# fanzhongyi/ExploreMultiModal

Hardware: AMD Instinct MI355X
Metric: image-text pairs/sec fwd+bwd, VLMo-Base, 1/2/4/8 MI355X; % bf16 MFMA roofline (higher is better)
Workload: dtype bf16

## Files before the change

exploremultimodal_amd/csrc/block.hip:

```cpp
#include "common.h"
#include "vlmo_hip.h"
#include <algorithm>
#include <map>
#include <vector>

namespace {
constexpr int GELU_DERIV = 4;


struct Events {
    std::vector<hipEvent_t> pool;
    hipEvent_t get(size_t i) {
        while (pool.size() <= i) {
            hipEvent_t e = nullptr;
            (void)hipEventCreateWithFlags(&e, hipEventDisableTiming);
            pool.push_back(e);
        }
        return pool[i];
    }
};
Events& events() {
    static thread_local std::map<int, Events> per_device;
    int dev = 0;
    (void)hipGetDevice(&dev);
// ... 152 lines not shown
    VLMO_CHECK_ARG(b->dx2 && b->dx1 && b->dx0, "vlmo_stack_bwd: block %d: null gradient buffers", i);
    VLMO_CHECK_ARG(b->n_experts >= 1 && b->n_experts <= 2 && b->n_attn >= 1 && b->n_attn <= 2,
                   "vlmo_stack_bwd: block %d: 1..2 experts and attention launches per block", i);
    VLMO_CHECK_ARG(b->M > 0 && b->exp_rows[0] >= 0 && (b->n_experts == 1 || b->exp_rows[1] >= 0) &&
                       (int64_t)b->exp_rows[0] + (b->n_experts == 2 ? b->exp_rows[1] : 0) <= b->M,
                   "vlmo_stack_bwd: block %d: expert rows exceed M = %d", i, b->M);
    const int64_t need = stack_ws_layout(b->M, b->d, b->hidden, block_seqs(b)).total * 4;
    VLMO_CHECK_ARG(b->ws_main && b->ws_bytes >= need,
                   "vlmo_stack_bwd: block %d: column workspace of %lld bytes is too small: need %lld bytes = "
                   "vlmo_stack_bwd_ws_bytes(%d, %d, %d, %d)",
                   i, (long long)b->ws_bytes, (long long)need, b->M, b->d, b->hidden, block_seqs(b));
    return 0;
}

int block_dgrad_chain(const VlmoBlockDesc* b, hipStream_t st, Deferred& D, const VlmoBlockDesc* below, bool skip_resid,
                      bool* fused_below) {
    const int M = b->M, d = b->d, hid = b->hidden;
    const int nseq_all = block_seqs(b);
    const StackWs W = stack_ws_layout(M, d, hid, nseq_all);
    const int64_t slot_bytes = W.slot * 4;
    float* const ws = b->ws_main;
    const void *ag[4], *wg[4], *af[4], *wf[4];
    int32_t rows[4];
    VlmoEpilogue eg[4], ef[4];
    float* colpart = ws + W.colpart;
    for (int x = 0; x < b->n_experts; ++x) {
        const size_t r0 = b->exp_row0[x];
        const int n = rows[x] = b->exp_rows[x];
        if (!skip_resid) {
            VlmoColJob fold{};
            TRY(resid_bwd_launch(b->dx2 + r0 * d, bp(b->zd2, r0, d, 2), b->g2,
// ... 49 lines not shown
                          b->dqkv, qvsum + (size_t)s0 * 2 * d, b->heads, d, b->maxlen[a], scale, b->attn_drop_thresh,
                          b->attn_inv_keep, b->seed + 11 + b->attn_seed_idx[a], b->attn_seq0[a], st));
    push_tn(D, b->dz1, d, b->ctx, d, b->dproj_w, d, M, d, d);
    push_tn(D, b->dqkv, 3 * d, b->y1, d, b->dqkv_w, d, M, 3 * d, d);
    push_col(D, fold_job(qvsum, 2 * d, nseq_all, 2 * d, d, b->dqkv_b, b->dqkv_b + 2 * d));
    {
        VlmoEpilogue e = epi();
        e.out = b->dy1;
        e.ldo = d;
        TRY(vlmo_gemm_nt(VLMO_EPI_BIAS, VLMO_BF16, b->tile, b->dqkv, 3 * d, b->qkv_wT, 3 * d, M, d, 3 * d, &e, st));
    }
    const VlmoBlockDesc* n = below;
    *fused_below = n && n->M == M && n->d == d && n->dx2 == b->dx0 && n->zd2 && n->dz2 && n->exp_row0[0] == 0 &&
                   (n->n_experts == 1 ? n->exp_rows[0] == M
                                      : (n->exp_row0[1] == n->exp_rows[0] && n->exp_rows[0] + n->exp_rows[1] == M));
    VlmoColJob fold{};
    if (*fused_below) {
        const int seg = n->n_experts == 1 ? M : n->exp_row0[1];
        float* wsf = ws + W.ln1;
        int nb0 = 0;
        TRY(ln_resid_seg_bwd(b->dy1, b->x, b->n1w, b->mean1, b->rstd1, b->dx1, b->dx0, b->dn1w, b->dn1b, n->zd2, n->g2,
                             n->rs2, n->row_index, n->dz2, n->dg2, n->drop_thresh, n->inv_keep, n->seed + 21, n->seed + 23,
                             seg, M, d, wsf, 2 * slot_bytes, &fold, &nb0, st));
        push_col(D, fold);
        if (n->db2[0]) push_col(D, fold_job(wsf + 3 * d, 4 * d, nb0, d, d, n->db2[0]));
        if (n->n_experts == 2 && n->db2[1])
            push_col(D, fold_job(wsf + 3 * d + (size_t)nb0 * 4 * d, 4 * d, fold.rows - nb0, d, d, n->db2[1]));
    } else {
        TRY(ln_bwd_fold(b->dy1, b->x, b->n1w, b->mean1, b->rstd1, b->dx1, b->dx0, b->dn1w, b->dn1b, nullptr, nullptr, nullptr,
                        nullptr, nullptr, nullptr, nullptr, 0, 1.f, 0, M, d, ws + W.ln1, slot_bytes, &fold, st));
        push_col(D, fold);
    }
    return 0;
}

}

extern "C" int64_t vlmo_stack_bwd_ws_bytes(int M, int d, int hidden, int max_seqs) {
    return stack_ws_layout(M, d, hidden, max_seqs).total * 4;
}

extern "C" int vlmo_stack_fwd(const VlmoStackDesc* s, hipStream_t st) {
    VLMO_CHECK_ARG(s && s->blocks && s->n_blocks >= 1, "vlmo_stack_fwd: empty stack");
    for (int i = 0; i < s->n_blocks; ++i)
        if (int rc = block_fwd(&s->blocks[i], st)) return rc;
    return 0;
}

extern "C" int vlmo_stack_bwd(const VlmoStackDesc* s, hipStream_t st) {
    VLMO_CHECK_ARG(s && s->blocks && s->n_blocks >= 1, "vlmo_stack_bwd: empty stack");
    const int nb = s->n_blocks;
    for (int i = 0; i < nb; ++i) TRY(check_block_bwd(&s->blocks[i], i));
    const int batch = s->wgrad_batch >= 1 ? s->wgrad_batch : 1;
    const int nsets = s->n_tmp_sets >= 1 ? s->n_tmp_sets : 1;
    hipStream_t side = s->side_stream ? s->side_stream : st;
    const bool two = side != st;
    VLMO_CHECK_ARG(!two || nsets > batch || nb <= nsets,
                   "vlmo_stack_bwd: %d temporary sets cannot cover deferred batches of %d blocks", nsets, batch);
    Events& ev = events();
    Deferred D;
    D.store = s->wgrad_store != 0;
    std::vector<int> batch_of(nb, -1);
    int n_batches = 0, waited_upto = -1;
    auto flush = [&]() -> int {
        if (D.blocks.empty()) return 0;
        if (two) {
            hipEvent_t f = ev.get(2 * n_batches);
            (void)hipEventRecord(f, st);
            (void)hipStreamWaitEvent(side, f, 0);
        }
        std::stable_sort(D.tn.begin(), D.tn.end(), [](const VlmoTnProblem& a, const VlmoTnProblem& b) { return a.M > b.M; });
        TRY(vlmo_gemm_tn_multi(VLMO_BF16, D.tn.data(), (int)D.tn.size(), side));
        TRY(vlmo_colwork_multi(VLMO_BF16, D.col.data(), (int)D.col.size(), side));
        if (two) (void)hipEventRecord(ev.get(2 * n_batches + 1), side);
        if (s->grad_ready)
            for (int i : D.blocks)
                if (s->grad_ready[i]) (void)hipEventRecord((hipEvent_t)s->grad_ready[i], side);
        ++n_batches;
        D.tn.clear();
        D.col.clear();
        D.blocks.clear();
        return 0;
    };
    auto set_free = [&](int kk) -> int {
        if (!two || kk < nsets || kk >= nb) return 0;
        int need = batch_of[kk - nsets];
        if (need < 0 || need >= n_batches) {
            TRY(flush());
            need = n_batches - 1;
        }
        if (need >= 0 && need > waited_upto) {
            (void)hipStreamWaitEvent(st, ev.get(2 * need + 1), 0);
            waited_upto = need;
        }
        return 0;
    };
    bool skip_resid = false;
    for (int k = 0; k < nb; ++k) {
        const int i = nb - 1 - k;
        TRY(set_free(k));
        TRY(set_free(k + 1));
        bool fused = false;
        TRY(block_dgrad_chain(&s->blocks[i], st, D, i > 0 ? &s->blocks[i - 1] : nullptr, skip_resid, &fused));
        skip_resid = fused;
        D.blocks.push_back(i);
        batch_of[k] = n_batches;
        if ((int)D.blocks.size() >= batch || k == nb - 1) TRY(flush());
    }
    if (two && n_batches > 0) (void)hipStreamWaitEvent(st, ev.get(2 * (n_batches - 1) + 1), 0);
    return 0;
}

extern "C" int vlmo_event_create(void** out) {
    VLMO_CHECK_ARG(out, "vlmo_event_create: null out");
    hipEvent_t e = nullptr;
    hipError_t rc = hipEventCreateWithFlags(&e, hipEventDisableTiming);
    if (rc != hipSuccess) {
        vlmo_set_error("vlmo_event_create: %s", hipGetErrorString(rc));
        return (int)rc;
    }
    *out = e;
    return 0;
// ... 7 lines not shown
```

exploremultimodal_amd/csrc/gemm_tn.hip:

```cpp
#include "gemm_common.h"
#include <algorithm>
#include <vector>

namespace {

struct GemmTN {
    const void* A;
    const void* B;
    float* C;
    int M, N1, N2, lda, ldb, ldc;
    int kt_per_split, tiles;
    float alpha;
    float* slab;
    int mode;
};
enum { TN_ATOMIC = 0, TN_ACCUM = 1, TN_STORE = 2 };

__device__ __attribute__((aligned(256))) char tn_zero_page[256];

__device__ __forceinline__ int tn_swz(int row) { return ((row & 3) << 2) | ((row >> 2) & 3); }

template <typename T, int BM, int BN, int WM, int WN, bool PP = false>
__device__ __forceinline__ void gemm_tn_body(const GemmTN& p, const int lid) {
    typedef typename Elem<T>::v8 v8;
// ... 225 lines not shown
                        p.slab[((size_t)split * p.N1 + gm) * p.N2 + gn] = acc[i][j][r];
                    else if (p.mode == TN_STORE)
                        *c = p.alpha * acc[i][j][r];
                    else
                        atomicAdd(c, p.alpha * acc[i][j][r]);
                }
            }
        }
}

template <typename T, int BM, int BN, int WM, int WN, bool PP = false>
__global__ __launch_bounds__(WM * WN * 64, 2) void gemm_tn_kernel(const GemmTN p) {
    gemm_tn_body<T, BM, BN, WM, WN, PP>(p, xcd_remap(blockIdx.x, gridDim.x));
}

constexpr int MAX_TN_PROBS = 16;
constexpr int MAX_TN_ORDER = 1024;
constexpr uint16_t TN_NOP = 0xFFFF;
struct GemmTNMulti {
    int n;
    GemmTN p[MAX_TN_PROBS];
    uint16_t order[MAX_TN_ORDER];
};
template <typename T>
__global__ __launch_bounds__(512, 2) void gemm_tn_multi_kernel(const GemmTNMulti mp) {
    const uint32_t code = mp.order[blockIdx.x];
    if (code == TN_NOP) return;
    int gi = (int)(code >> 12);
    const int lid_in = __builtin_amdgcn_readfirstlane((int)(code & 0xFFFu));
    gi = __builtin_amdgcn_readfirstlane(gi);
    const GemmTN& q = mp.p[gi];
    GemmTN p;
    p.A = uniform_ptr(q.A), p.B = uniform_ptr(q.B), p.C = (float*)uniform_ptr(q.C);
    p.M = __builtin_amdgcn_readfirstlane(q.M), p.N1 = __builtin_amdgcn_readfirstlane(q.N1);
    p.N2 = __builtin_amdgcn_readfirstlane(q.N2), p.lda = __builtin_amdgcn_readfirstlane(q.lda);
    p.ldb = __builtin_amdgcn_readfirstlane(q.ldb), p.ldc = __builtin_amdgcn_readfirstlane(q.ldc);
    p.kt_per_split = __builtin_amdgcn_readfirstlane(q.kt_per_split), p.tiles = __builtin_amdgcn_readfirstlane(q.tiles);
    p.alpha = __builtin_bit_cast(float, __builtin_amdgcn_readfirstlane(__builtin_bit_cast(int, q.alpha)));
    p.slab = nullptr;
    p.mode = __builtin_amdgcn_readfirstlane(q.mode);
    gemm_tn_body<T, 256, 256, 2, 4, true>(p, lid_in);
}

__global__ __launch_bounds__(256) void tn_reduce_kernel(const float* __restrict__ slab, int splits, int N1, int N2,
                                                        float* __restrict__ C, int ldc, float alpha) {
    const int n4 = N2 >> 2;
// ... 21 lines not shown
    int splits = splits_req;
    if (splits <= 0) {
        if (pl.big) {
            splits = 256 / pl.tiles;
        } else {
            splits = 512 / pl.tiles;
            if (splits < 4) splits = 1024 / pl.tiles;
        }
        if (splits < 1) splits = 1;
    }
    if (splits > nk) splits = nk;
    pl.per = (nk + splits - 1) / splits;
    pl.splits = (nk + pl.per - 1) / pl.per;
    return pl;
}
}

extern "C" int64_t vlmo_gemm_tn_ws_bytes(int M, int N1, int N2) {
    const TnPlan a = tn_plan(M, N1, N2, 0, 0);
    return (int64_t)a.splits * N1 * N2 * 4;
}

extern "C" int vlmo_gemm_tn(int dtype, const void* A, int lda, const void* B, int ldb, float* C, int ldc,
                            int M, int N1, int N2, float alpha, int splits, float* ws, int64_t ws_bytes,
                            hipStream_t stream) {
    VLMO_CHECK_ARG(A && B && C, "vlmo_gemm_tn: null operand");
    VLMO_CHECK_ARG(M > 0 && N1 >= 8 && N2 >= 8, "vlmo_gemm_tn: bad problem M=%d N1=%d N2=%d", M, N1, N2);
    VLMO_CHECK_ARG(N1 % 8 == 0 && N2 % 8 == 0 && lda % 8 == 0 && ldb % 8 == 0, "vlmo_gemm_tn: N1,N2,lda,ldb must be multiples of 8");
    VLMO_CHECK_ARG(lda >= N1 && ldb >= N2 && ldc >= N2, "vlmo_gemm_tn: leading dimension too small");
    VLMO_CHECK_ARG(dtype == VLMO_BF16 || dtype == VLMO_F16, "vlmo_gemm_tn: dtype must be bf16 or f16");
// ... 54 lines not shown
        }
        long tiles_all = 0;
        int min_nk = 1 << 30;
        double flops = 0;
        for (int q = 0; q < nq; ++q) {
            const VlmoTnProblem& r = probs[q0 + q];
            VLMO_CHECK_ARG(r.A && r.B && r.C, "vlmo_gemm_tn_multi: null operand in problem %d", q0 + q);
            VLMO_CHECK_ARG(r.M > 0 && r.N1 >= 8 && r.N2 >= 8 && r.N1 % 8 == 0 && r.N2 % 8 == 0 && r.lda % 8 == 0 &&
                               r.ldb % 8 == 0 && r.lda >= r.N1 && r.ldb >= r.N2 && r.ldc >= r.N2,
                           "vlmo_gemm_tn_multi: bad shape in problem %d (M=%d N1=%d N2=%d)", q0 + q, r.M, r.N1, r.N2);
            tiles_all += (long)((r.N1 + 255) / 256) * ((r.N2 + 255) / 256);
            const int nk = (r.M + 63) / 64;
            if (nk < min_nk) min_nk = nk;
            flops += 2.0 * r.M * r.N1 * r.N2;
        }
        int splits = 1;
        if (tiles_all < 192) {
            splits = (int)(256 / tiles_all);
            if (splits > min_nk / 8) splits = min_nk / 8;
            if (splits < 1) splits = 1;
        }
        GemmTNMulti mp{};
        mp.n = nq;
        struct Job {
            uint16_t code;
            int cost;
        };
        std::vector<Job> jobs;
        for (int q = 0; q < nq; ++q) {
            const VlmoTnProblem& r = probs[q0 + q];
            const int tiles = ((r.N1 + 255) / 256) * ((r.N2 + 255) / 256);
            const int nk = (r.M + 63) / 64;
            int sp = splits > nk ? nk : splits;
            const int per = (nk + sp - 1) / sp;
            sp = (nk + per - 1) / per;
            int mode = r.accumulate ? TN_ACCUM : TN_STORE;
            if (sp > 1) {
                mode = TN_ATOMIC;
                if (!r.accumulate) {
                    hipError_t rc = hipMemset2DAsync(r.C, (size_t)r.ldc * 4, 0, (size_t)r.N2 * 4, r.N1, stream);
                    if (rc != hipSuccess) {
                        vlmo_set_error("vlmo_gemm_tn_multi: memset failed: %s", hipGetErrorString(rc));
                        return (int)rc;
                    }
                }
            }
            VLMO_CHECK_ARG(tiles * sp <= 4096, "vlmo_gemm_tn_multi: problem %d has too many tiles", q0 + q);
            mp.p[q] = GemmTN{r.A, r.B, r.C, r.M, r.N1, r.N2, r.lda, r.ldb, r.ldc, per, tiles, r.alpha, nullptr, mode};
            for (int l = 0; l < tiles * sp; ++l) jobs.push_back(Job{(uint16_t)((q << 12) | l), per});
        }
        std::stable_sort(jobs.begin(), jobs.end(), [](const Job& a, const Job& b) { return a.cost > b.cost; });
        std::vector<uint16_t> bins[8];
        for (size_t i = 0; i < jobs.size();) {
            size_t j = i;
            while (j < jobs.size() && jobs[j].cost == jobs[i].cost) ++j;
            const size_t cnt = j - i;
            for (int x = 0; x < 8; ++x)
                for (size_t k = i + cnt * x / 8; k < i + cnt * (x + 1) / 8; ++k) bins[x].push_back(jobs[k].code);
            i = j;
        }
        size_t deepest = 0;
        for (int x = 0; x < 8; ++x) deepest = bins[x].size() > deepest ? bins[x].size() : deepest;
        VLMO_CHECK_ARG(deepest * 8 <= (size_t)MAX_TN_ORDER, "vlmo_gemm_tn_multi: %zu workgroups exceed one launch (pass fewer problems per call)",
                       jobs.size());
        const int t = (int)deepest * 8;
        for (int b = 0; b < t; ++b) {
            const std::vector<uint16_t>& bin = bins[b & 7];
            mp.order[b] = (size_t)(b >> 3) < bin.size() ? bin[b >> 3] : TN_NOP;
        }
        ProfScope prof(73, flops, stream);
        constexpr int LDS = 2 * 4 * 64 * 256;
        if (dtype == VLMO_F16)
            hipLaunchKernelGGL((gemm_tn_multi_kernel<f16>), dim3(t), dim3(512), LDS, stream, mp);
        else
// ... 6 lines not shown
```

exploremultimodal_amd/engine.py:

```python
import ctypes
import os as _os
import sys
from collections import namedtuple

import torch

from . import hip

LN_EPS = 1e-12
GRAD_SINK = None
_ov = _os.environ.get('VLMO_OVERLAP_WGRAD')
OVERLAP_WGRAD = None if _ov is None else _ov != '0'
ONE_STREAM_ROWS = 12288


def _use_side_stream(sink, rows):
    if OVERLAP_WGRAD is not None:
        return OVERLAP_WGRAD
    return sink is not None or rows < ONE_STREAM_ROWS


DEFAULT_TILE = -1


# ... 421 lines not shown

def wgrad_batch_for(d, hid, cus=256, max_batch=4):
    if WGRAD_BATCH > 0:
        return WGRAD_BATCH
    c = lambda n: -(-n // 256)
    tiles = c(d) * c(3 * d) + c(d) * c(d) + 2 * c(d) * c(hid)
    best, best_cost = 1, None
    for b in range(1, max_batch + 1):
        cost = -(-b * tiles // cus) / b
        if best_cost is None or cost < best_cost - 1e-9:
            best, best_cost = b, cost
    return best


TMP_SETS = 4
USE_STACK = True

_PERSIST = {}


def _persist(dev, tag, numel, dtype):
    key = (dev, torch.cuda.current_stream(dev).cuda_stream, tag)
    t = _PERSIST.get(key)
    if t is None or t.numel() < numel or t.dtype != dtype:
        t = _PERSIST[key] = torch.empty(numel, dtype=dtype, device=dev)
    return t


_EVENTS = {}

# ... 330 lines not shown
                                          storage, off)
            store_ok = store_ok and all(fr for _, fr in got)
            acquired += [(f_, fr, g.lo > 0) for g, (f_, fr) in zip(blk, got)]
            grads = _fill_grads(D, [f_ for f_, _ in got], d, hid, len(blk) - 1)
            for g, (_, fr) in zip(blk, got):
                if fr or sink is not None:
                    grads_all[o + g.lo:o + g.hi] = grads[g.lo:g.hi]
            _split_backward_attention(D, metas[i])
            _wire_temporaries(D, k, nb, M * d, sc, dxo, dx_in)
        _zero_buckets(acquired, store_ok, d, hid)
        S = hip.StackDesc()
        S.n_blocks, S.wgrad_batch, S.n_tmp_sets, S.wgrad_store = nb, sc.batch, sc.nsets, int(store_ok)
        S.blocks = ctypes.cast(descs, ctypes.POINTER(hip.BlockDesc))
        side = _side_stream(dev) if _use_side_stream(sink, M) else None
        S.side_stream = side.cuda_stream if side is not None else None
        evs = None
        if sink is not None and side is not None:
            evs = _ready_events(dev, nb)
            arr = (ctypes.c_void_p * nb)(*evs)
            S.grad_ready = ctypes.cast(arr, ctypes.POINTER(ctypes.c_void_p))
        hip.stack_bwd(S)
        if any(mt.capture is not None for mt in metas):
            _run_captures(metas, ctx.keep[0], sc, M, d)
        ctx.descs = ctx.keep = None
        if sink is not None:
            _hand_to_sink(sink, groups, spans, grads_all, evs)
            return (dx_in, None) + (None,) * len(params)
        return (dx_in, None, *grads_all)


# ... 109 lines not shown
```

exploremultimodal_amd/hip.py:

```python
import ctypes
import os

import numpy as np
import torch

_HERE = os.path.dirname(os.path.abspath(__file__))
LIB_PATH = os.environ.get('VLMO_HIP_LIB') or os.path.join(_HERE, 'lib', 'libvlmo_hip.so')

BF16, F16, F32 = 0, 1, 2
EPI_BIAS, EPI_BIAS_GELU, EPI_RESID, EPI_DGELU, EPI_F32, EPI_DUAL, EPI_ARGMAX, EPI_CE, EPI_CE_BWD = 0, 1, 2, 3, 4, 5, 6, 7, 8

_vp, _i32, _u32, _u64, _f32, _i64 = (ctypes.c_void_p, ctypes.c_int32, ctypes.c_uint32,
                                     ctypes.c_uint64, ctypes.c_float, ctypes.c_int64)


class Epilogue(ctypes.Structure):
    _fields_ = [('out', _vp), ('out2', _vp), ('bias', _vp), ('gamma', _vp),
                ('resid', _vp), ('row_scale', _vp), ('row_index', _vp), ('aux', _vp),
                ('ldo', _i32), ('ld2', _i32), ('relu', _i32),
                ('drop_thresh', _u32), ('inv_keep', _f32), ('beta', _f32),
                ('seed', _u64), ('colpart', _vp)]


_fp = _vp
# ... 11 lines not shown
        + [(n, _fp) for n in ('g1', 'g2', 'n1w', 'n1b', 'n2w', 'n2b', 'qkv_bias', 'proj_b',
                              'qkv_w', 'qkv_wT', 'proj_w', 'proj_wT')]
        + [(n, _fp * 2) for n in ('b1', 'b2', 'w1', 'w1T', 'w2', 'w2T')]
        + [(n, _fp) for n in ('x', 'x1', 'x2', 'y1', 'qkv', 'ctx', 'zd1', 'y2', 'u', 'h', 'zd2',
                              'mean1', 'rstd1', 'mean2', 'rstd2')]
        + [('lse', _fp * 2)]
        + [(n, _fp) for n in ('dx2', 'dx1', 'dx0', 'dz2', 'du', 'dy2', 'dz1', 'dctx', 'dqkv', 'dy1',
                              'dg1', 'dg2', 'dn1w', 'dn1b', 'dn2w', 'dn2b', 'dqkv_w', 'dqkv_b',
                              'dproj_w', 'dproj_b')]
        + [(n, _fp * 2) for n in ('dw1', 'db1', 'dw2', 'db2')]
        + [('ws_main', _fp), ('ws_bytes', _i64)])


class StackDesc(ctypes.Structure):
    _fields_ = [('n_blocks', _i32), ('wgrad_batch', _i32), ('n_tmp_sets', _i32), ('wgrad_store', _i32),
                ('blocks', ctypes.POINTER(BlockDesc)), ('side_stream', _vp), ('grad_ready', ctypes.POINTER(_vp))]


class TnProblem(ctypes.Structure):
    _fields_ = [('A', _vp), ('B', _vp), ('C', _vp), ('lda', _i32), ('ldb', _i32), ('ldc', _i32),
                ('M', _i32), ('N1', _i32), ('N2', _i32), ('alpha', _f32), ('accumulate', _i32)]


class ColJob(ctypes.Structure):
    _fields_ = [('kind', _i32), ('ld', _i32), ('src', _vp), ('rows', _i32), ('ncols', _i32),
                ('out', _vp * 4), ('n0', _i32), ('pad_', _i32)]


class Image(ctypes.Structure):
    _fields_ = [('offset', _i64), ('H', _i32), ('W', _i32)]


class AugSlot(ctypes.Structure):
    _fields_ = [('op', _i32), ('pad_', _i32), ('a', ctypes.c_double), ('b', ctypes.c_double)]


# ... 33 lines not shown
                         ctypes.POINTER(Epilogue), _vp],
    'vlmo_dvae_im2col': [_vp, _vp, _i32, _i32, _i32, _i32, _i32, _i32, _vp],
    'vlmo_maxpool2_nhwc': [_vp, _vp, _vp, _i32, _i32, _i32, _i32, _vp],
    'vlmo_argmax_reduce': [_vp, _i32, _vp, _i32, _vp],
    'vlmo_dvae_embed': [_vp, _vp, _vp, _vp, _i32, _i32, _i32, _vp],
    'vlmo_upsample2_nhwc': [_vp, _vp, _i32, _i32, _i32, _i32, _vp],
    'vlmo_dvae_out_head': [_vp, _vp, _vp, _vp, _i32, _i32, _i32, _i32, _i32, _vp],
    'vlmo_conv4s2_nhwc': [_i32, _vp, _i32, _i32, _i32, _i32, _vp, _i32, _vp, ctypes.POINTER(Epilogue), _vp],
    'vlmo_convt4s2_nhwc': [_i32, _vp, _i32, _i32, _i32, _i32, _vp, _i32, _vp, ctypes.POINTER(Epilogue), _vp],
    'vlmo_dvae_patch4s2': [_vp, _vp, _i32, _i32, _i32, _i32, _i32, _vp],
    'vlmo_dvae_out_head_linear': [_vp, _vp, _vp, _vp, _i32, _i32, _i32, _i32, _i32, _vp],
    'vlmo_ce_reduce': [_vp, _i32, _vp, _i32, _vp, _vp, _vp, _i32, _vp],
    'vlmo_stack_fwd': [ctypes.POINTER(StackDesc), _vp],
    'vlmo_stack_bwd': [ctypes.POINTER(StackDesc), _vp],
    'vlmo_gemm_tn_multi': [_i32, ctypes.POINTER(TnProblem), _i32, _vp],
    'vlmo_colwork_multi': [_i32, ctypes.POINTER(ColJob), _i32, _vp],
    'vlmo_event_create': [ctypes.POINTER(ctypes.c_void_p)],
    'vlmo_event_destroy': [_vp],
    'vlmo_stream_wait_event': [_vp, _vp],
    'vlmo_profile_start': [_i32],
    'vlmo_gemm_nt_grouped': [_i32, _i32, _i32, _i32, _vp, _i32, _vp, _i32, _vp, _i32, _i32, _vp, _vp],
    'vlmo_mt_grad_norm': [ctypes.c_void_p, _f32, _f32, _vp, _vp, _vp],
    'vlmo_mt_adam': [ctypes.c_void_p, ctypes.c_void_p, _vp, _vp],
    'vlmo_mt_ema': [ctypes.c_void_p, _f32, _vp],
    'vlmo_mt_adam_ema': [ctypes.c_void_p, ctypes.c_void_p, _vp, _vp, _f32, _vp],
    'vlmo_side_stream_create': [_i32, ctypes.POINTER(ctypes.c_uint32), _i32, ctypes.POINTER(ctypes.c_void_p)],
    'vlmo_profile_stop': [_i32, ctypes.POINTER(ctypes.c_double), ctypes.POINTER(ctypes.c_double),
                          ctypes.POINTER(ctypes.c_int64)],
    'vlmo_gemm_nt_2src': [_i32, _i32, _i32, _vp, _i32, _i32, _f32, _vp, _i32, _vp, _i32, _i32, _i32, _i32,
                          ctypes.POINTER(Epilogue), _vp],
# ... 9 lines not shown
    'vlmo_grad_unpack': [_vp, _vp, _i64, _vp],
    'vlmo_ln_gelu_fwd': [_vp, _i32, _vp, _vp, _vp, _i32, _vp, _vp, _i32, _i32, _f32, _vp],
    'vlmo_ln_gelu_bwd': [_vp, _i32, _vp, _i32, _vp, _vp, _vp, _vp, _vp, _i32, _vp, _i32, _vp, _vp, _vp, _i32, _i32, _vp,
                         _i64, _vp],
    'vlmo_vqa_bce': [_vp, _i32, _vp, _i32, _i32, _i32, _vp, _vp, _vp, _vp, _f32, _vp, _i32, _vp, _i32, _vp],
    'vlmo_isda_update': [_vp, _i32, _vp, _vp, _vp, _vp, _vp, _i32, _i32, _i32, _i32, _vp, _vp, _vp, _vp, _vp],
    'vlmo_isda_aug_fwd': [_vp, _i32, _vp, _vp, _i32, _i32, _i32, _i32, _f32, _vp, _i32, _vp, _i64, _vp],
    'vlmo_isda_aug_bwd': [_vp, _i32, _vp, _i32, _vp, _vp, _i32, _i32, _i32, _i32, _f32, _vp, _i32, _vp, _i64, _vp],
    'vlmo_sim_topk': [_vp, _i32, _vp, _i32, _i32, _i32, _i32, _i32, _f32, _i32, _vp, ctypes.c_size_t, _vp, _vp, _vp],
    'vlmo_crop_resample': [_vp, _i64, _vp, _vp, _i32, _vp, _vp, _i32, ctypes.POINTER(_f32), ctypes.POINTER(_f32), _f32, _vp,
                           _i64, _vp],
    'vlmo_randaug': [_vp, _vp, _vp, _i64, _vp, _vp, _i32, _vp, _vp, _i32, _i32, _vp, _i64, _vp],
}

_lib = None
ABI_VERSION = 15

def lib():
    global _lib
    if _lib is None:
        if not os.path.exists(LIB_PATH):
            raise RuntimeError(
                f'{LIB_PATH} not found: build the HIP extension first '
                '(python -c "import __graft_entry__ as g; g.build()" or '
                'make -C exploremultimodal_amd/csrc). There is no CPU fallback.')
        L = ctypes.CDLL(LIB_PATH)
        L.vlmo_last_error.restype = ctypes.c_char_p
        L.vlmo_abi_version.restype = ctypes.c_int
        if L.vlmo_abi_version() != ABI_VERSION:
            raise RuntimeError(f'{LIB_PATH} has ABI version {L.vlmo_abi_version()}, this package needs {ABI_VERSION}: '
                               'rebuild it (make -C exploremultimodal_amd/csrc)')
        L.vlmo_reduce_ws_bytes.restype = ctypes.c_int64
        L.vlmo_reduce_ws_bytes.argtypes = [_i32]
        L.vlmo_stack_bwd_ws_bytes.restype = ctypes.c_int64
        L.vlmo_stack_bwd_ws_bytes.argtypes = [_i32, _i32, _i32, _i32]
        L.vlmo_gemm_tn_ws_bytes.restype = ctypes.c_int64
        L.vlmo_isda_ws_bytes.restype = ctypes.c_int64
        L.vlmo_isda_ws_bytes.argtypes = [_i32, _i32, _i32]
        L.vlmo_gemm_tn_ws_bytes.argtypes = [_i32, _i32, _i32]
        L.vlmo_sim_topk_ws_bytes.restype = ctypes.c_int64
        L.vlmo_sim_topk_ws_bytes.argtypes = [_i32, _i32, _i32, _i32]
        L.vlmo_randaug_ws_bytes.restype = ctypes.c_int64
        L.vlmo_randaug_ws_bytes.argtypes = [_i32]
        L.vlmo_embed_txt_rows_ws_bytes.restype = ctypes.c_int64
        L.vlmo_embed_txt_rows_ws_bytes.argtypes = [_i32, _i32, _i32]
        for name, sig in _SIGS.items():
            fn = getattr(L, name)
            fn.argtypes = sig
            fn.restype = ctypes.c_int
        _lib = L
    return _lib


def exported_symbols():
    return ['vlmo_last_error', 'vlmo_abi_version', 'vlmo_reduce_ws_bytes', 'vlmo_stack_bwd_ws_bytes',
            'vlmo_gemm_tn_ws_bytes', 'vlmo_isda_ws_bytes', 'vlmo_sim_topk_ws_bytes', 'vlmo_randaug_ws_bytes',
            'vlmo_embed_txt_rows_ws_bytes'] + list(_SIGS)


def _check(rc, name):
    if rc != 0:
        raise RuntimeError(f'{name} failed (rc={rc}): {lib().vlmo_last_error().decode()}')


def _p(t):
    return None if t is None else t.data_ptr()


def _stream():
    return torch.cuda.current_stream().cuda_stream


# ... 284 lines not shown
    _check(lib().vlmo_dvae_patch4s2(_p(x), _p(out), B, C, H, W, Kpad, _stream()), 'vlmo_dvae_patch4s2')


def dvae_out_head_linear(x, w, bias, out, B, H, W):
    Cout, C = w.shape
    _check(lib().vlmo_dvae_out_head_linear(_p(x), _p(w), _p(bias), _p(out), B, H, W, C, Cout, _stream()),
           'vlmo_dvae_out_head_linear')


def gemm_tn_multi(problems, dtype=BF16):
    n = len(problems)
    arr = (TnProblem * n)()
    for i, (A, B, C, M, N1, N2, acc) in enumerate(problems):
        arr[i] = TnProblem(_p(A), _p(B), _p(C), A.stride(0), B.stride(0), C.stride(0), M, N1, N2, 1.0, int(acc))
    _check(lib().vlmo_gemm_tn_multi(dtype, arr, n, _stream()), 'vlmo_gemm_tn_multi')


def colwork_multi(jobs, dtype=BF16):
    n = len(jobs)
    arr = (ColJob * n)()
    for i, (kind, src, rows, ncols, outs, n0) in enumerate(jobs):
        o = (ctypes.c_void_p * 4)(*[_p(t) for t in (list(outs) + [None] * 4)[:4]])
        arr[i] = ColJob(kind, src.stride(0), _p(src), rows, ncols, o, n0, 0)
    _check(lib().vlmo_colwork_multi(dtype, arr, n, _stream()), 'vlmo_colwork_multi')


def event_create():
    out = ctypes.c_void_p()
    _check(lib().vlmo_event_create(ctypes.byref(out)), 'vlmo_event_create')
    return out.value
# ... 288 lines not shown
```

include/vlmo_hip.h:

```cpp
#ifndef VLMO_HIP_H
#define VLMO_HIP_H

#include <stddef.h>
#include <stdint.h>

#ifdef __cplusplus
extern "C" {
#endif

#ifndef __HIP_PLATFORM_AMD__
typedef struct ihipStream_t* hipStream_t;
#endif

enum { VLMO_BF16 = 0, VLMO_F16 = 1, VLMO_F32 = 2 };

enum {
    VLMO_EPI_BIAS = 0,
    VLMO_EPI_BIAS_GELU = 1,
    VLMO_EPI_RESID = 2,
    VLMO_EPI_DGELU = 3,
    VLMO_EPI_F32 = 4,
    VLMO_EPI_DUAL = 5,
    VLMO_EPI_ARGMAX = 6,
    VLMO_EPI_CE = 7,
// ... 7 lines not shown
    const float* gamma;
    const float* resid;
    const float* row_scale;
    const int32_t* row_index;
    const void* aux;
    int32_t ldo, ld2;
    int32_t relu;
    uint32_t drop_thresh;
    float inv_keep;
    float beta;
    uint64_t seed;
    float* colpart;
} VlmoEpilogue;

const char* vlmo_last_error(void);
#define VLMO_ABI_VERSION 15
int vlmo_abi_version(void);

int vlmo_gemm_nt(int epi, int dtype, int tile, const void* A, int lda, const void* B, int ldb,
                 int M, int N, int K, const VlmoEpilogue* e, hipStream_t stream);
int vlmo_gemm_nt_2src(int epi, int dtype, int tile, const void* A, int lda, int k1, float seg_scale, const void* A2,
                      int lda2, const void* B, int ldb, int M, int N, int K, const VlmoEpilogue* e,
                      hipStream_t stream);
int vlmo_gemm_nt_grouped(int epi, int dtype, int tile, int ngroups, const void* const* A, int lda,
                         const void* const* B, int ldb, const int32_t* M, int N, int K,
                         const VlmoEpilogue* e, hipStream_t stream);

int64_t vlmo_gemm_tn_ws_bytes(int M, int N1, int N2);
int vlmo_gemm_tn(int dtype, const void* A, int lda, const void* B, int ldb, float* C, int ldc,
                 int M, int N1, int N2, float alpha, int splits, float* ws, int64_t ws_bytes,
                 hipStream_t stream);

typedef struct VlmoTnProblem {
    const void* A;
    const void* B;
    float* C;
    int32_t lda, ldb, ldc;
    int32_t M, N1, N2;
    float alpha;
    int32_t accumulate;
} VlmoTnProblem;
int vlmo_gemm_tn_multi(int dtype, const VlmoTnProblem* probs, int n, hipStream_t stream);

int vlmo_ln_fwd(const float* x, const float* w, const float* b, void* y, int out_f32,
                float* mean, float* rstd, const int32_t* rowmap, int M, int d, float eps,
                hipStream_t stream);
int64_t vlmo_reduce_ws_bytes(int ncols);

int vlmo_ln_bwd(const void* dy, int dy_f32, const int32_t* rowmap, const float* x, const float* w,
                const float* mean, const float* rstd, const float* dres, float* dx, float* dw,
                float* db, int M, int d, float* ws, int64_t ws_bytes, hipStream_t stream);

int vlmo_ln_resid_bwd(const void* dy, const float* x, const float* w, const float* mean, const float* rstd,
                      const float* dres, float* dx, float* dw, float* db, const void* zd, const float* gamma,
                      const float* row_scale, const int32_t* row_index, void* dz, float* dgamma, float* dbias,
                      uint32_t drop_thresh, float inv_keep, uint64_t seed, int M, int d, float* ws,
                      int64_t ws_bytes, hipStream_t stream);
// ... 125 lines not shown
    const float* dx2;
    float *dx1, *dx0;
    void *dz2, *du, *dy2, *dz1, *dctx, *dqkv, *dy1;
    float *dg1, *dg2, *dn1w, *dn1b, *dn2w, *dn2b, *dqkv_w, *dqkv_b, *dproj_w, *dproj_b;
    float *dw1[2], *db1[2], *dw2[2], *db2[2];
    float* ws_main;
    int64_t ws_bytes;
} VlmoBlockDesc;

typedef struct VlmoStackDesc {
    int32_t n_blocks, wgrad_batch, n_tmp_sets;
    int32_t wgrad_store;
    const VlmoBlockDesc* blocks;
    hipStream_t side_stream;
    void* const* grad_ready;
} VlmoStackDesc;
int64_t vlmo_stack_bwd_ws_bytes(int M, int d, int hidden, int max_seqs);
int vlmo_stack_fwd(const VlmoStackDesc* s, hipStream_t stream);
int vlmo_stack_bwd(const VlmoStackDesc* s, hipStream_t stream);
int vlmo_event_create(void** out);
int vlmo_event_destroy(void* ev);
int vlmo_stream_wait_event(hipStream_t stream, void* ev);

#define VLMO_COMM_ID_BYTES 128
int vlmo_comm_available(void);
int vlmo_comm_unique_id(void* id128);
int vlmo_comm_init(void** comm, const void* id128, int rank, int world);
int vlmo_comm_destroy(void* comm);
int vlmo_comm_count(void* comm, int* ranks, int* rank);
int vlmo_comm_all_reduce(void* comm, const void* send, void* recv, int64_t count, int dtype, hipStream_t stream);
// ... 118 lines not shown
```

Before: 4565.

## Add wgrad carry planning across batches and bin-packed XCD ordering for TN GEMM

Adds an optional mode that splits deferred weight-gradient TN GEMMs along the reduction dimension. The head of each problem runs in the current batch and the tail is carried into the next batch's launch. A cost-model planner, cached by shape, picks the cut points to balance workgroup makespan across XCDs. The multi-TN launcher now always reorders each XCD's jobs with a bin-packing heuristic, shrinks the per-problem argument struct, and raises the problem limit. The carry mode is off by default, so only the reordering and the struct change affect the default path.

```diff
diff --git a/exploremultimodal_amd/csrc/block.hip b/exploremultimodal_amd/csrc/block.hip
--- a/exploremultimodal_amd/csrc/block.hip
+++ b/exploremultimodal_amd/csrc/block.hip
@@ -1,7 +1,9 @@
 #include "common.h"
 #include "vlmo_hip.h"
 #include <algorithm>
+#include <functional>
 #include <map>
+#include <mutex>
 #include <vector>
 
 namespace {
@@ -190,7 +192,7 @@
 }
 
 int block_dgrad_chain(const VlmoBlockDesc* b, hipStream_t st, Deferred& D, const VlmoBlockDesc* below, bool skip_resid,
-                      bool* fused_below) {
+                      bool* fused_below, const std::function<int()>* before_last = nullptr) {
     const int M = b->M, d = b->d, hid = b->hidden;
     const int nseq_all = block_seqs(b);
     const StackWs W = stack_ws_layout(M, d, hid, nseq_all);
@@ -270,6 +272,7 @@
     *fused_below = n && n->M == M && n->d == d && n->dx2 == b->dx0 && n->zd2 && n->dz2 && n->exp_row0[0] == 0 &&
                    (n->n_experts == 1 ? n->exp_rows[0] == M
                                       : (n->exp_row0[1] == n->exp_rows[0] && n->exp_rows[0] + n->exp_rows[1] == M));
+    if (before_last) TRY((*before_last)());
     VlmoColJob fold{};
     if (*fused_below) {
         const int seg = n->n_experts == 1 ? M : n->exp_row0[1];
@@ -290,6 +293,31 @@
     return 0;
 }
 
+int tn_carry_plan_cached(const std::vector<VlmoTnShape>& probs, const std::vector<VlmoTnShape>& carried, int allow_cut,
+                         int32_t* cut_rows, float* makespan) {
+    struct Plan {
+        std::vector<int32_t> cut;
+        float span;
+    };
+    static std::mutex mu;
+    static std::map<std::vector<int32_t>, Plan> cache;
+    std::vector<int32_t> key{allow_cut, (int32_t)probs.size()};
+    for (const VlmoTnShape& p : probs) key.insert(key.end(), {p.M, p.N1, p.N2});
+    for (const VlmoTnShape& p : carried) key.insert(key.end(), {p.M, p.N1, p.N2});
+    std::lock_guard<std::mutex> lock(mu);
+    auto it = cache.find(key);
+    if (it == cache.end()) {
+        Plan pl{std::vector<int32_t>(probs.size(), 0), 0.f};
+        TRY(vlmo_tn_carry_plan(probs.data(), (int)probs.size(), carried.data(), (int)carried.size(), 256, 0.f, allow_cut,
+                               pl.cut.data(), &pl.span));
+        if (cache.size() > 256) cache.clear();
+        it = cache.emplace(key, pl).first;
+    }
+    if (cut_rows) std::copy(it->second.cut.begin(), it->second.cut.end(), cut_rows);
+    *makespan = it->second.span;
+    return 0;
+}
+
 }
 
 extern "C" int64_t vlmo_stack_bwd_ws_bytes(int M, int d, int hidden, int max_seqs) {
@@ -318,6 +346,47 @@
     D.store = s->wgrad_store != 0;
     std::vector<int> batch_of(nb, -1);
     int n_batches = 0, waited_upto = -1;
+    const bool carry = s->wgrad_carry && !two && !s->grad_ready && (nsets >= 2 * batch || nb <= nsets);
+    std::vector<VlmoTnProblem> carried;
+    bool tn_issued = false, last_batch = false;
+    auto flush_tn = [&]() -> int {
+        tn_issued = true;
+        std::stable_sort(D.tn.begin(), D.tn.end(), [](const VlmoTnProblem& a, const VlmoTnProblem& b) { return a.M > b.M; });
+        if (!carry) return vlmo_gemm_tn_multi(VLMO_BF16, D.tn.data(), (int)D.tn.size(), side);
+        const int n = (int)D.tn.size();
+        auto shapes = [](const std::vector<VlmoTnProblem>& v) {
+            std::vector<VlmoTnShape> o;
+            for (const VlmoTnProblem& p : v) o.push_back(VlmoTnShape{p.M, p.N1, p.N2});
+            return o;
+        };
+        const std::vector<VlmoTnShape> sh = shapes(D.tn), in = shapes(carried);
+        std::vector<int32_t> cut(n, 0);
+        float span = 0.f;
+        TRY(tn_carry_plan_cached(sh, in, last_batch ? 2 : 1, cut.data(), &span));
+        std::vector<VlmoTnProblem> tails;
+        for (int q = 0; q < n; ++q)
+            if (cut[q] > 0) {
+                VlmoTnProblem t = D.tn[q];
+                t.A = (const char*)t.A + (size_t)cut[q] * t.lda * 2;
+                t.B = (const char*)t.B + (size_t)cut[q] * t.ldb * 2;
+                t.M -= cut[q];
+                t.accumulate = 1;
+                tails.push_back(t);
+            }
+        std::vector<VlmoTnProblem> launch;
+        for (int q = 0; q < n; ++q) {
+            launch.push_back(D.tn[q]);
+            if (cut[q] > 0) launch.back().M = cut[q];
+        }
+        launch.insert(launch.end(), carried.begin(), carried.end());
+        TRY(vlmo_gemm_tn_multi(VLMO_BF16, launch.data(), (int)launch.size(), side));
+        carried.swap(tails);
+        if (last_batch && !carried.empty()) {
+            TRY(vlmo_gemm_tn_multi(VLMO_BF16, carried.data(), (int)carried.size(), side));
+            carried.clear();
+        }
+        return 0;
+    };
     auto flush = [&]() -> int {
         if (D.blocks.empty()) return 0;
         if (two) {
@@ -325,8 +394,8 @@
             (void)hipEventRecord(f, st);
             (void)hipStreamWaitEvent(side, f, 0);
         }
-        std::stable_sort(D.tn.begin(), D.tn.end(), [](const VlmoTnProblem& a, const VlmoTnProblem& b) { return a.M > b.M; });
-        TRY(vlmo_gemm_tn_multi(VLMO_BF16, D.tn.data(), (int)D.tn.size(), side));
+        if (!tn_issued) TRY(flush_tn());
+        tn_issued = false;
         TRY(vlmo_colwork_multi(VLMO_BF16, D.col.data(), (int)D.col.size(), side));
         if (two) (void)hipEventRecord(ev.get(2 * n_batches + 1), side);
         if (s->grad_ready)
@@ -357,11 +426,15 @@
         TRY(set_free(k));
         TRY(set_free(k + 1));
         bool fused = false;
-        TRY(block_dgrad_chain(&s->blocks[i], st, D, i > 0 ? &s->blocks[i - 1] : nullptr, skip_resid, &fused));
+        const bool ends_batch = (int)D.blocks.size() + 1 >= batch || k == nb - 1;
+        last_batch = k == nb - 1;
+        const std::function<int()> early = flush_tn;
+        TRY(block_dgrad_chain(&s->blocks[i], st, D, i > 0 ? &s->blocks[i - 1] : nullptr, skip_resid, &fused,
+                              carry && ends_batch ? &early : nullptr));
         skip_resid = fused;
         D.blocks.push_back(i);
         batch_of[k] = n_batches;
-        if ((int)D.blocks.size() >= batch || k == nb - 1) TRY(flush());
+        if (ends_batch) TRY(flush());
     }
     if (two && n_batches > 0) (void)hipStreamWaitEvent(st, ev.get(2 * (n_batches - 1) + 1), 0);
     return 0;
diff --git a/exploremultimodal_amd/csrc/gemm_tn.hip b/exploremultimodal_amd/csrc/gemm_tn.hip
--- a/exploremultimodal_amd/csrc/gemm_tn.hip
+++ b/exploremultimodal_amd/csrc/gemm_tn.hip
@@ -1,5 +1,6 @@
 #include "gemm_common.h"
 #include <algorithm>
+#include <functional>
 #include <vector>
 
 namespace {
@@ -263,22 +264,34 @@
     gemm_tn_body<T, BM, BN, WM, WN, PP>(p, xcd_remap(blockIdx.x, gridDim.x));
 }
 
-constexpr int MAX_TN_PROBS = 16;
+constexpr int MAX_TN_PROBS = 24;
+constexpr int TN_LID_BITS = 11;
 constexpr int MAX_TN_ORDER = 1024;
 constexpr uint16_t TN_NOP = 0xFFFF;
+struct GemmTNArg {
+    const void* A;
+    const void* B;
+    float* C;
+    int M, N1, N2, lda, ldb, ldc;
+    int kt_per_split, tiles;
+    float alpha;
+    int mode;
+};
 struct GemmTNMulti {
     int n;
-    GemmTN p[MAX_TN_PROBS];
+    GemmTNArg p[MAX_TN_PROBS];
     uint16_t order[MAX_TN_ORDER];
 };
+static_assert(sizeof(GemmTNArg) == 64 && sizeof(GemmTNMulti) <= 4096, "the launch table must fit one argument block");
+static_assert(MAX_TN_PROBS <= (0xFFFF >> TN_LID_BITS), "problem index and TN_NOP share the 16-bit placement code");
 template <typename T>
 __global__ __launch_bounds__(512, 2) void gemm_tn_multi_kernel(const GemmTNMulti mp) {
     const uint32_t code = mp.order[blockIdx.x];
     if (code == TN_NOP) return;
-    int gi = (int)(code >> 12);
-    const int lid_in = __builtin_amdgcn_readfirstlane((int)(code & 0xFFFu));
+    int gi = (int)(code >> TN_LID_BITS);
+    const int lid_in = __builtin_amdgcn_readfirstlane((int)(code & ((1u << TN_LID_BITS) - 1)));
     gi = __builtin_amdgcn_readfirstlane(gi);
-    const GemmTN& q = mp.p[gi];
+    const GemmTNArg& q = mp.p[gi];
     GemmTN p;
     p.A = uniform_ptr(q.A), p.B = uniform_ptr(q.B), p.C = (float*)uniform_ptr(q.C);
     p.M = __builtin_amdgcn_readfirstlane(q.M), p.N1 = __builtin_amdgcn_readfirstlane(q.N1);
@@ -330,6 +343,226 @@
     pl.splits = (nk + pl.per - 1) / pl.per;
     return pl;
 }
+
+int tn_multi_splits(long tiles_all, int min_nk) {
+    int splits = 1;
+    if (tiles_all < 192) {
+        splits = (int)(256 / tiles_all);
+        if (splits > min_nk / 8) splits = min_nk / 8;
+        if (splits < 1) splits = 1;
+    }
+    return splits;
+}
+
+constexpr double TN_JOB_FIXED = 2.0;
+constexpr double TN_TAIL_FACTOR = 1.8;
+constexpr int TN_MIN_PART = 16;
+
+double tn_xcd_makespan(const std::vector<int>& order, const std::vector<double>& dur, int ncu) {
+    std::vector<double> cu(ncu, 0.0);
+    for (int i : order) {
+        std::pop_heap(cu.begin(), cu.end(), std::greater<double>());
+        cu.back() += dur[i];
+        std::push_heap(cu.begin(), cu.end(), std::greater<double>());
+    }
+    return *std::max_element(cu.begin(), cu.end());
+}
+std::vector<int> tn_xcd_order(const std::vector<double>& cost, int ncu) {
+    const int n = (int)cost.size();
+    std::vector<int> order(n);
+    for (int i = 0; i < n; ++i) order[i] = i;
+    if (n <= ncu) return order;
+    const double lpt = tn_xcd_makespan(order, cost, ncu);
+    double sum = 0.0;
+    for (double c : cost) sum += c;
+    double lo = std::max(cost[0], sum / ncu), hi = lpt;
+    std::vector<double> start(n), best_start;
+    auto pack = [&](double cap) {
+        std::vector<double> load(ncu, 0.0);
+        for (int i = 0; i < n; ++i) {
+            int b = 0;
+            while (b < ncu && load[b] + cost[i] > cap + 1e-9) ++b;
+            if (b == ncu) return false;
+            start[i] = load[b];
+            load[b] += cost[i];
+        }
+        return true;
+    };
+    if (pack(lo)) {
+        best_start = start;
+    } else {
+        for (int it = 0; it < 12; ++it) {
+            const double mid = 0.5 * (lo + hi);
+            if (pack(mid)) hi = mid, best_start = start;
+            else lo = mid;
+        }
+    }
+    if (best_start.empty()) return order;
+    std::vector<int> packed = order;
+    std::stable_sort(packed.begin(), packed.end(), [&](int a, int b) { return best_start[a] < best_start[b]; });
+    return tn_xcd_makespan(packed, cost, ncu) < lpt - 1e-9 ? packed : order;
+}
+
+struct PlanJob {
+    int kt, tiles;
+    bool tail;
+};
+inline int tn_tiles(int N1, int N2) { return ((N1 + 255) / 256) * ((N2 + 255) / 256); }
+
+double tn_launch_makespan(const std::vector<PlanJob>& jobs, int cus, double factor, int* splits_out = nullptr) {
+    if (splits_out) *splits_out = 1;
+    if (jobs.empty()) return 0.0;
+    if ((int)jobs.size() > MAX_TN_PROBS) return -1.0;
+    long tiles_all = 0;
+    int min_nk = 1 << 30;
+    for (const PlanJob& j : jobs) tiles_all += j.tiles, min_nk = std::min(min_nk, j.kt);
+    const int splits = tn_multi_splits(tiles_all, min_nk);
+    if (splits_out) *splits_out = splits;
+    struct W {
+        int per;
+        double dur;
+    };
+    std::vector<W> w;
+    for (const PlanJob& j : jobs) {
+        int sp = std::min(splits, j.kt);
+        const int per = (j.kt + sp - 1) / sp;
+        sp = (j.kt + per - 1) / per;
+        for (int l = 0; l < j.tiles * sp; ++l) w.push_back(W{per, per * (j.tail ? factor : 1.0) + TN_JOB_FIXED});
+    }
+    std::stable_sort(w.begin(), w.end(), [](const W& a, const W& b) { return a.per > b.per; });
+    std::vector<double> cost[8], dur[8];
+    for (size_t i = 0; i < w.size();) {
+        size_t j = i;
+        while (j < w.size() && w[j].per == w[i].per) ++j;
+        const size_t cnt = j - i;
+        for (int x = 0; x < 8; ++x)
+            for (size_t k = i + cnt * x / 8; k < i + cnt * (x + 1) / 8; ++k) {
+                cost[x].push_back(w[k].per + TN_JOB_FIXED);
+                dur[x].push_back(w[k].dur);
+            }
+        i = j;
+    }
+    const int per_xcd = std::max(1, cus / 8);
+    double worst = 0.0;
+    for (int x = 0; x < 8; ++x) {
+        if (cost[x].size() * 8 > (size_t)MAX_TN_ORDER) return -1.0;
+        if (x > 0 && cost[x] == cost[x - 1] && dur[x] == dur[x - 1]) continue;
+        worst = std::max(worst, tn_xcd_makespan(tn_xcd_order(cost[x], per_xcd), dur[x], per_xcd));
+    }
+    return worst;
+}
+}
+
+extern "C" void vlmo_tn_carry_limits(int32_t* max_problems, int32_t* max_workgroups, int32_t* arg_bytes) {
+    if (max_problems) *max_problems = MAX_TN_PROBS;
+    if (max_workgroups) *max_workgroups = MAX_TN_ORDER;
+    if (arg_bytes) *arg_bytes = (int32_t)sizeof(GemmTNMulti);
+}
+
+extern "C" int vlmo_tn_carry_plan(const VlmoTnShape* probs, int n, const VlmoTnShape* carried, int n_carried, int cus,
+                                  float tail_factor, int allow_cut, int32_t* cut_rows, float* makespan) {
+    VLMO_CHECK_ARG(n >= 0 && n_carried >= 0 && (n == 0 || probs) && (n_carried == 0 || carried) && (n == 0 || cut_rows),
+                   "vlmo_tn_carry_plan: null argument");
+    if (cus <= 0) cus = 256;
+    const double factor = tail_factor > 0.f ? (double)tail_factor : TN_TAIL_FACTOR;
+    auto nk_of = [](int M) { return (M + 63) / 64; };
+    for (int q = 0; q < n; ++q) {
+        VLMO_CHECK_ARG(probs[q].M > 0 && probs[q].N1 > 0 && probs[q].N2 > 0, "vlmo_tn_carry_plan: bad shape in problem %d", q);
+        cut_rows[q] = 0;
+    }
+    std::vector<PlanJob> in;
+    for (int q = 0; q < n_carried; ++q) {
+        VLMO_CHECK_ARG(carried[q].M > 0 && carried[q].N1 > 0 && carried[q].N2 > 0, "vlmo_tn_carry_plan: bad carried shape %d", q);
+        in.push_back(PlanJob{nk_of(carried[q].M), tn_tiles(carried[q].N1, carried[q].N2), true});
+    }
+    int cls[2] = {0, 0}, ncls = 0;
+    auto launches = [&](const int* hl, double* now, double* next) {
+        std::vector<PlanJob> a = in, b;
+        for (int q = 0; q < n; ++q) {
+            const int nk = nk_of(probs[q].M), t = tn_tiles(probs[q].N1, probs[q].N2);
+            int h = 0;
+            for (int c = 0; c < ncls; ++c)
+                if (cls[c] == nk) h = hl[c];
+            a.push_back(PlanJob{h ? h : nk, t, false});
+            b.push_back(PlanJob{h ? h : nk, t, false});
+            if (h) b.push_back(PlanJob{nk - h, t, true});
+        }
+        *now = tn_launch_makespan(a, cus, factor);
+        *next = tn_launch_makespan(b, cus, factor);
+    };
+    const int none[2] = {0, 0};
+    double now = 0, next = 0;
+    launches(none, &now, &next);
+    if (now < 0) {
+        if (makespan) *makespan = -1.f;
+        return 0;
+    }
+    int best[2] = {0, 0};
+    double best_cost = now, best_now = now;
+    long tiles_all = 0;
+    int min_nk = 1 << 30;
+    for (int q = 0; q < n; ++q) tiles_all += tn_tiles(probs[q].N1, probs[q].N2), min_nk = std::min(min_nk, nk_of(probs[q].M));
+    if (allow_cut && n > 0 && tn_multi_splits(tiles_all, min_nk) == 1) {
+        for (int q = 0; q < n && ncls < 2; ++q) {
+            int pick = 0;
+            for (int r = 0; r < n; ++r) {
+                const int nk = nk_of(probs[r].M);
+                if (nk >= 2 * TN_MIN_PART && (ncls == 0 || nk < cls[ncls - 1]) && nk > pick) pick = nk;
+            }
+            if (!pick) break;
+            cls[ncls++] = pick;
+        }
+        auto heads_of = [&](const int* hl) { return (hl[0] ? hl[0] : cls[0]) + (ncls > 1 ? (hl[1] ? hl[1] : cls[1]) : 0); };
+        auto consider = [&](int h0, int h1) {
+            const int hl[2] = {h0, h1};
+            if (!h0 && !h1) return;
+            double a, b;
+            launches(hl, &a, &b);
+            if (a < 0 || b < 0) return;
+            const double cost = std::max(a, b);
+            if (cost > 0.97 * now) return;
+            const bool have = best[0] || best[1];
+            if (!have || cost < best_cost - 1e-9 || (cost < best_cost + 1e-9 && heads_of(hl) > heads_of(best)))
+                best_cost = cost, best_now = a, best[0] = h0, best[1] = h1;
+        };
+        auto range = [&](int c, int step, int around) {
+            std::vector<int> v{0};
+            if (c >= ncls) return v;
+            int lo = std::max(TN_MIN_PART, (cls[c] + 1) / 2), hi = cls[c] - TN_MIN_PART;
+            if (around) lo = std::max(lo, around - 3), hi = std::min(hi, around + 3);
+            for (int h = lo; h <= hi; h += step) v.push_back(h);
+            return v;
+        };
+        if (ncls > 0) {
+            const int step = cls[0] > 64 ? 4 : 1;
+            for (int h0 : range(0, step, 0))
+                for (int h1 : range(1, step, 0)) consider(h0, h1);
+            if (step > 1 && (best[0] || best[1])) {
+                const std::vector<int> r0 = best[0] ? range(0, 1, best[0]) : std::vector<int>{0};
+                const std::vector<int> r1 = best[1] ? range(1, 1, best[1]) : std::vector<int>{0};
+                for (int h0 : r0)
+                    for (int h1 : r1) consider(h0, h1);
+            }
+        }
+        if (allow_cut == 2 && (best[0] || best[1])) {
+            std::vector<PlanJob> t;
+            for (int q = 0; q < n; ++q)
+                for (int c = 0; c < ncls; ++c)
+                    if (cls[c] == nk_of(probs[q].M) && best[c])
+                        t.push_back(PlanJob{cls[c] - best[c], tn_tiles(probs[q].N1, probs[q].N2), true});
+            int sp = 1;
+            const double rest = tn_launch_makespan(t, cus, factor, &sp);
+            if (rest < 0 || sp > 1 || now <= best_now + rest)
+                best[0] = best[1] = 0, best_now = now;
+            else
+                best_now += rest;
+        }
+        for (int q = 0; q < n; ++q)
+            for (int c = 0; c < ncls; ++c)
+                if (cls[c] == nk_of(probs[q].M) && best[c]) cut_rows[q] = best[c] * 64;
+    }
+    if (makespan) *makespan = (float)best_now;
+    return 0;
 }
 
 extern "C" int64_t vlmo_gemm_tn_ws_bytes(int M, int N1, int N2) {
@@ -414,12 +647,7 @@
             if (nk < min_nk) min_nk = nk;
             flops += 2.0 * r.M * r.N1 * r.N2;
         }
-        int splits = 1;
-        if (tiles_all < 192) {
-            splits = (int)(256 / tiles_all);
-            if (splits > min_nk / 8) splits = min_nk / 8;
-            if (splits < 1) splits = 1;
-        }
+        const int splits = tn_multi_splits(tiles_all, min_nk);
         GemmTNMulti mp{};
         mp.n = nq;
         struct Job {
@@ -445,19 +673,29 @@
                     }
                 }
             }
-            VLMO_CHECK_ARG(tiles * sp <= 4096, "vlmo_gemm_tn_multi: problem %d has too many tiles", q0 + q);
-            mp.p[q] = GemmTN{r.A, r.B, r.C, r.M, r.N1, r.N2, r.lda, r.ldb, r.ldc, per, tiles, r.alpha, nullptr, mode};
-            for (int l = 0; l < tiles * sp; ++l) jobs.push_back(Job{(uint16_t)((q << 12) | l), per});
+            VLMO_CHECK_ARG(tiles * sp <= (1 << TN_LID_BITS), "vlmo_gemm_tn_multi: problem %d has too many tiles", q0 + q);
+            mp.p[q] = GemmTNArg{r.A, r.B, r.C, r.M, r.N1, r.N2, r.lda, r.ldb, r.ldc, per, tiles, r.alpha, mode};
+            for (int l = 0; l < tiles * sp; ++l) jobs.push_back(Job{(uint16_t)((q << TN_LID_BITS) | l), per});
         }
         std::stable_sort(jobs.begin(), jobs.end(), [](const Job& a, const Job& b) { return a.cost > b.cost; });
         std::vector<uint16_t> bins[8];
+        std::vector<double> cost[8];
         for (size_t i = 0; i < jobs.size();) {
             size_t j = i;
             while (j < jobs.size() && jobs[j].cost == jobs[i].cost) ++j;
             const size_t cnt = j - i;
             for (int x = 0; x < 8; ++x)
-                for (size_t k = i + cnt * x / 8; k < i + cnt * (x + 1) / 8; ++k) bins[x].push_back(jobs[k].code);
+                for (size_t k = i + cnt * x / 8; k < i + cnt * (x + 1) / 8; ++k) {
+                    bins[x].push_back(jobs[k].code);
+                    cost[x].push_back(jobs[k].cost + TN_JOB_FIXED);
+                }
             i = j;
+        }
+        for (int x = 0; x < 8; ++x) {
+            const std::vector<int> ord = tn_xcd_order(cost[x], 256 / 8);
+            std::vector<uint16_t> b(bins[x].size());
+            for (size_t k = 0; k < ord.size(); ++k) b[k] = bins[x][ord[k]];
+            bins[x].swap(b);
         }
         size_t deepest = 0;
         for (int x = 0; x < 8; ++x) deepest = bins[x].size() > deepest ? bins[x].size() : deepest;
diff --git a/exploremultimodal_amd/engine.py b/exploremultimodal_amd/engine.py
--- a/exploremultimodal_amd/engine.py
+++ b/exploremultimodal_amd/engine.py
@@ -459,6 +459,7 @@
 
 
 TMP_SETS = 4
+WGRAD_CARRY = False
 USE_STACK = True
 
 _PERSIST = {}
@@ -819,6 +820,7 @@
         S.blocks = ctypes.cast(descs, ctypes.POINTER(hip.BlockDesc))
         side = _side_stream(dev) if _use_side_stream(sink, M) else None
         S.side_stream = side.cuda_stream if side is not None else None
+        S.wgrad_carry = int(WGRAD_CARRY)
         evs = None
         if sink is not None and side is not None:
             evs = _ready_events(dev, nb)
diff --git a/exploremultimodal_amd/hip.py b/exploremultimodal_amd/hip.py
--- a/exploremultimodal_amd/hip.py
+++ b/exploremultimodal_amd/hip.py
@@ -49,12 +49,17 @@
 
 class StackDesc(ctypes.Structure):
     _fields_ = [('n_blocks', _i32), ('wgrad_batch', _i32), ('n_tmp_sets', _i32), ('wgrad_store', _i32),
-                ('blocks', ctypes.POINTER(BlockDesc)), ('side_stream', _vp), ('grad_ready', ctypes.POINTER(_vp))]
+                ('blocks', ctypes.POINTER(BlockDesc)), ('side_stream', _vp), ('grad_ready', ctypes.POINTER(_vp)),
+                ('wgrad_carry', _i32)]
 
 
 class TnProblem(ctypes.Structure):
     _fields_ = [('A', _vp), ('B', _vp), ('C', _vp), ('lda', _i32), ('ldb', _i32), ('ldc', _i32),
                 ('M', _i32), ('N1', _i32), ('N2', _i32), ('alpha', _f32), ('accumulate', _i32)]
+
+
+class TnShape(ctypes.Structure):
+    _fields_ = [('M', _i32), ('N1', _i32), ('N2', _i32)]
 
 
 class ColJob(ctypes.Structure):
@@ -118,6 +123,8 @@
     'vlmo_stack_fwd': [ctypes.POINTER(StackDesc), _vp],
     'vlmo_stack_bwd': [ctypes.POINTER(StackDesc), _vp],
     'vlmo_gemm_tn_multi': [_i32, ctypes.POINTER(TnProblem), _i32, _vp],
+    'vlmo_tn_carry_plan': [ctypes.POINTER(TnShape), _i32, ctypes.POINTER(TnShape), _i32, _i32, _f32, _i32,
+                           ctypes.POINTER(_i32), ctypes.POINTER(_f32)],
     'vlmo_colwork_multi': [_i32, ctypes.POINTER(ColJob), _i32, _vp],
     'vlmo_event_create': [ctypes.POINTER(ctypes.c_void_p)],
     'vlmo_event_destroy': [_vp],
@@ -157,7 +164,7 @@
 }
 
 _lib = None
-ABI_VERSION = 15
+ABI_VERSION = 16
 
 def lib():
     global _lib
@@ -187,6 +194,8 @@
         L.vlmo_randaug_ws_bytes.argtypes = [_i32]
         L.vlmo_embed_txt_rows_ws_bytes.restype = ctypes.c_int64
         L.vlmo_embed_txt_rows_ws_bytes.argtypes = [_i32, _i32, _i32]
+        L.vlmo_tn_carry_limits.restype = None
+        L.vlmo_tn_carry_limits.argtypes = [ctypes.POINTER(_i32)] * 3
         for name, sig in _SIGS.items():
             fn = getattr(L, name)
             fn.argtypes = sig
@@ -198,7 +207,7 @@
 def exported_symbols():
     return ['vlmo_last_error', 'vlmo_abi_version', 'vlmo_reduce_ws_bytes', 'vlmo_stack_bwd_ws_bytes',
             'vlmo_gemm_tn_ws_bytes', 'vlmo_isda_ws_bytes', 'vlmo_sim_topk_ws_bytes', 'vlmo_randaug_ws_bytes',
-            'vlmo_embed_txt_rows_ws_bytes'] + list(_SIGS)
+            'vlmo_embed_txt_rows_ws_bytes', 'vlmo_tn_carry_limits'] + list(_SIGS)
 
 
 def _check(rc, name):
@@ -513,6 +522,21 @@
     for i, (A, B, C, M, N1, N2, acc) in enumerate(problems):
         arr[i] = TnProblem(_p(A), _p(B), _p(C), A.stride(0), B.stride(0), C.stride(0), M, N1, N2, 1.0, int(acc))
     _check(lib().vlmo_gemm_tn_multi(dtype, arr, n, _stream()), 'vlmo_gemm_tn_multi')
+
+
+def tn_carry_plan(problems, carried=(), cus=0, tail_factor=0.0, allow_cut=True):
+    n, m = len(problems), len(carried)
+    pa, ca = (TnShape * max(n, 1))(*[TnShape(*p) for p in problems]), (TnShape * max(m, 1))(*[TnShape(*c) for c in carried])
+    cuts, span = (_i32 * max(n, 1))(), _f32()
+    _check(lib().vlmo_tn_carry_plan(pa, n, ca, m, cus, tail_factor, int(allow_cut), cuts, ctypes.byref(span)),
+           'vlmo_tn_carry_plan')
+    return list(cuts[:n]), span.value
+
+
+def tn_carry_limits():
+    a, b, c = _i32(), _i32(), _i32()
+    lib().vlmo_tn_carry_limits(ctypes.byref(a), ctypes.byref(b), ctypes.byref(c))
+    return a.value, b.value, c.value
 
 
 def colwork_multi(jobs, dtype=BF16):
diff --git a/include/vlmo_hip.h b/include/vlmo_hip.h
--- a/include/vlmo_hip.h
+++ b/include/vlmo_hip.h
@@ -45,7 +45,7 @@
 } VlmoEpilogue;
 
 const char* vlmo_last_error(void);
-#define VLMO_ABI_VERSION 15
+#define VLMO_ABI_VERSION 16
 int vlmo_abi_version(void);
 
 int vlmo_gemm_nt(int epi, int dtype, int tile, const void* A, int lda, const void* B, int ldb,
@@ -72,6 +72,13 @@
     int32_t accumulate;
 } VlmoTnProblem;
 int vlmo_gemm_tn_multi(int dtype, const VlmoTnProblem* probs, int n, hipStream_t stream);
+
+typedef struct VlmoTnShape {
+    int32_t M, N1, N2;
+} VlmoTnShape;
+int vlmo_tn_carry_plan(const VlmoTnShape* probs, int n, const VlmoTnShape* carried, int n_carried, int cus,
+                       float tail_factor, int allow_cut, int32_t* cut_rows, float* makespan);
+void vlmo_tn_carry_limits(int32_t* max_problems, int32_t* max_workgroups, int32_t* arg_bytes);
 
 int vlmo_ln_fwd(const float* x, const float* w, const float* b, void* y, int out_f32,
                 float* mean, float* rstd, const int32_t* rowmap, int M, int d, float eps,
@@ -227,6 +234,7 @@
     const VlmoBlockDesc* blocks;
     hipStream_t side_stream;
     void* const* grad_ready;
+    int32_t wgrad_carry;
 } VlmoStackDesc;
 int64_t vlmo_stack_bwd_ws_bytes(int M, int d, int hidden, int max_seqs);
 int vlmo_stack_fwd(const VlmoStackDesc* s, hipStream_t stream);
```

New measurement: 4539. No clear change (-0.6%).
